# nhcha6/embodied-object-detection

Hardware: AMD Instinct MI355X
Metric: frames/sec (640x640, implicit_memory); frames/sec/GPU = value / n_gpus (higher is better)
Workload: dtype f32

## Files before the change

embodied_object_detection_amd/csrc/conv_common.h:

```cpp
#pragma once
#include "eod_common.h"
#include "../../include/eod_hip.h"

namespace eodconv {


struct ConvArgs {
  const float* x;
  const float* w;
  const float* bias;
  const float* res;
  const float* gate;
  float* y;
  float* partial;
  const int* m_count;
  int m_unit;
  int m_segs, seg_rows;
  const float* fuse_w;
  const int* out_units;
  float fuse_b;
  int N, H, W, Cin, OH, OW, Cout, KH, KW, stride, pad, Kpad;
  int M, nchunks, splitk, cps;
  int relu, res_mode, in_relu, out_mode;
  int tiles_m, tiles_n;
  float out_scale;
  int nlv;
  int lv_off[EOD_MAX_LEVELS + 1], lv_h[EOD_MAX_LEVELS], lv_w[EOD_MAX_LEVELS];
  unsigned x_bytes, w_bytes;
  const void* w3;
  unsigned w3_bytes;
  const void* wh;
  unsigned wh_bytes;
  double* gn_partial;
  int gn_groups;
  float* y2;
  int split_n;
  FastDiv div_ow, div_oh, div_cd, div_row;
};

__device__ __forceinline__ int conv_row_limit(const ConvArgs& p, int M) {
  if (p.m_count && p.m_segs <= 1) {
    const int lim = *p.m_count * p.m_unit;
    M = lim < M ? lim : M;
  }
  return M;
}

__device__ __forceinline__ bool conv_row_active(const ConvArgs& p, int m) {
  if (!p.m_count || p.m_segs <= 1) return true;
  const int s = m / p.seg_rows;
  return m - s * p.seg_rows < p.m_count[s] * p.m_unit;
}

__device__ __forceinline__ bool conv_tile_active(const ConvArgs& p, int m0, int bm) {
  if (!p.m_count || p.m_segs <= 1) return true;
  const int last = (m0 + bm - 1 < p.M ? m0 + bm - 1 : p.M - 1);
  const int s0 = m0 / p.seg_rows, s1 = last / p.seg_rows;
  if (m0 - s0 * p.seg_rows < p.m_count[s0] * p.m_unit) return true;
  for (int s = s0 + 1; s <= s1; ++s)
    if (p.m_count[s] > 0) return true;
  return false;
}

template <bool GATE = false>
__device__ __forceinline__ float epilogue_store(const ConvArgs& p, float v, int m, int n) {
  int co = n;
  size_t oidx;
  if (p.out_mode == 1) {
    const int Cd = p.Cout >> 2;
    const int quad = (int)fdiv((unsigned)n, p.div_cd);
    co = n - quad * Cd;
    const int dy = quad >> 1, dx = quad & 1;
    const int t = (int)fdiv((unsigned)m, p.div_ow);
    const int ox = m - t * p.OW;
    const int img = (int)fdiv((unsigned)t, p.div_oh);
    const int oy = t - img * p.OH;
    oidx = ((size_t)(img * 2 * p.OH + 2 * oy + dy) * (2 * p.OW) + (2 * ox + dx)) * Cd + co;
  } else {
    oidx = (size_t)m * p.Cout + n;
  }
  if (p.bias) v += p.bias[co];
  v *= p.out_scale;
  if (p.res_mode == 1) {
    v += p.res[(size_t)m * p.Cout + n];
  } else if (p.res_mode == 2) {
    const int t = (int)fdiv((unsigned)m, p.div_ow);
    const int ox = m - t * p.OW;
    const int img = (int)fdiv((unsigned)t, p.div_oh);
    const int oy = t - img * p.OH;
    const int rh = p.OH >> 1, rw = p.OW >> 1;
    v += p.res[((size_t)(img * rh + (oy >> 1)) * rw + (ox >> 1)) * p.Cout + n];
  }
  if (p.split_n > 0) {
    if (n >= p.split_n) {
      if (p.relu) v = fmaxf(v, 0.0f);
      p.y2[(size_t)m * (p.Cout - p.split_n) + (n - p.split_n)] = v;
    } else {
      p.y[(size_t)m * p.split_n + n] = v;
    }
    return v;
  }
  if (p.relu) v = fmaxf(v, 0.0f);
  if (GATE && p.gate && !(p.gate[oidx] > 0.0f)) v = 0.0f;
  p.y[oidx] = v;
  return v;
}

__device__ __forceinline__ unsigned long long tap_mask(int iy0, int ix0, int hh, int ww, int KH, int KW) {
  unsigned long long mask = 0;
  int tp = 0;
  for (int ky = 0; ky < KH; ++ky) {
    const bool rok = (unsigned)(iy0 + ky) < (unsigned)hh;
    for (int kx = 0; kx < KW; ++kx, ++tp) {
      const bool ok = rok && ((unsigned)(ix0 + kx) < (unsigned)ww);
      mask |= (unsigned long long)ok << tp;
    }
  }
  return mask;
}

template <int TM, int TN, bool GATE = false>
__device__ __forceinline__ void store_wave_tiles(const ConvArgs& p, const f32x16 (&acc)[TM][TN], int m_base, int n_base, int M, int z,
                                                 int lane) {
  const int half = lane >> 5;
#pragma unroll
  for (int i = 0; i < TM; ++i) {
#pragma unroll
    for (int j = 0; j < TN; ++j) {
      const int n = n_base + j * 32 + (lane & 31);
#pragma unroll
      for (int r = 0; r < 16; ++r) {
        const int row = (r & 3) + 8 * (r >> 2) + 4 * half;
        const int m = m_base + i * 32 + row;
        if (m < M && n < p.Cout && conv_row_active(p, m)) {
          const float v = acc[i][j][r];
          if (p.splitk > 1) {
            p.partial[((size_t)z * p.M + m) * p.Cout + n] = v;
          } else {
            epilogue_store<GATE>(p, v, m, n);
          }
        }
      }
    }
  }
}

void launch_conv_fp32(const ConvArgs& a, int tile, int bk, bool tap4, dim3 grid, hipStream_t s, int lds_reserve = 0, int prefetch2 = 0);
void launch_conv_bf16x3(const ConvArgs& a, int tile, dim3 grid, hipStream_t s);
void launch_conv_wavek(const ConvArgs& a, int nw, dim3 grid, hipStream_t s);
void launch_split_weights(const float* w, void* out, int Cout, int Kpad, hipStream_t s);
void launch_conv_f16(const ConvArgs& a, int tile, int bk, dim3 grid, hipStream_t s);
void launch_half_weights(const float* w, void* out, int Cout, int Kpad, hipStream_t s);

}
```

embodied_object_detection_amd/csrc/conv_fp32.hip:

```cpp
#include "conv_operands.h"

namespace eodconv {
namespace {

template <int BM, int BN, int BK, bool TAP4, bool MULTI, int PIPE = 0>
__global__ __launch_bounds__(256) void conv_igemm_kernel(ConvArgs p) {
  constexpr bool PF2 = PIPE == 1;
  constexpr bool DB = PIPE == 2;
  constexpr int LS = BK + 4;
  constexpr int TM = BM / 64, TN = BN / 64;
  constexpr int QPR = BK / 4;
  constexpr int RPP = 256 / QPR;
  constexpr int AR = BM / RPP, BR = BN / RPP;
  static_assert(!TAP4 || BK == 32, "the stem path stages one 7x7 tap per float4: BK must be 32");
  constexpr int BUF = (BM + BN) * LS;
  __shared__ __attribute__((aligned(16))) float lds[(DB ? 2 : 1) * BUF];
  float* As = lds;
  float* Bs = lds + BM * LS;

  const int tid = threadIdx.x;
  const int lane = tid & 63;
  const int wave = tid >> 6;
  const int wm = wave >> 1, wn = wave & 1;

  int M;
  const int t = conv_first_tile<BM>(p, M);
  if (t < 0) return;
  const int tile_m = t / p.tiles_n;
  const int tile_n = t - tile_m * p.tiles_n;
  const int m0 = tile_m * BM, n0 = tile_n * BN;
  if (!conv_tile_active(p, m0, BM)) return;
  const int z = blockIdx.y;
  int c_end;
  const int c_begin = conv_chunk_range(p, p.cps, z, c_end);

  const int lr = tid / QPR, lq = tid % QPR;
  int a_off[AR], a_iy[AR], a_ix[AR];
  unsigned a_voff[AR];
  unsigned long long a_mask[AR];
  unsigned a_pitch[MULTI ? AR : 1];
#pragma unroll
  for (int i = 0; i < AR; ++i) {
    const int m = m0 + lr + RPP * i;
    const bool rowok = m < M;
    const RowOrigin o = conv_row_origin<MULTI>(p, m, rowok);
    a_iy[i] = rowok ? o.iy0 : -(1 << 28);
    a_ix[i] = o.ix0;
    a_off[i] = o.off;
    if (!TAP4) conv_row_address<MULTI>(p, o, rowok, lq, a_voff[i], a_mask[i], a_pitch[MULTI ? i : 0]);
  }
  unsigned w_voff[BR];
#pragma unroll
  for (int j = 0; j < BR; ++j) w_voff[j] = conv_w_row_offset(p, n0 + lr + RPP * j, lq);
  const __amdgpu_buffer_rsrc_t rsrc_x = conv_buffer(p.x, p.x_bytes);
  const __amdgpu_buffer_rsrc_t rsrc_w = conv_buffer(p.w, p.w_bytes);

  f32x4 ar0[AR], br0[BR];
  f32x4 ar1[PF2 ? AR : 1], br1[PF2 ? BR : 1];
  ChunkWalker<BK, MULTI> walk(p, c_begin);
  auto load_chunk = [&](int chunk, auto& ar, auto& br) {
    const int k0 = chunk * BK;
    if (!TAP4) {
      const TapInfo ti = walk.next(p);
#pragma unroll
      for (int i = 0; i < AR; ++i) ar[i] = conv_load_a<MULTI>(rsrc_x, ti, a_voff[i], a_mask[i], a_pitch[MULTI ? i : 0]);
    } else {
      const int tap = chunk * 8 + lq;
      const int ky = tap / p.KW;
      const int kx = tap - ky * p.KW;
      const bool tv = tap < p.KH * p.KW;
#pragma unroll
      for (int i = 0; i < AR; ++i) {
        const int iy = a_iy[i] + ky, ix = a_ix[i] + kx;
        const bool ok = tv && ((unsigned)iy < (unsigned)p.H) && ((unsigned)ix < (unsigned)p.W);
        f32x4 v = {0.f, 0.f, 0.f, 0.f};
        if (ok) v = *reinterpret_cast<const f32x4*>(p.x + (size_t)(a_off[i] + iy * p.W + ix) * 4);
        ar[i] = v;
      }
    }
    if (p.in_relu) {
#pragma unroll
      for (int i = 0; i < AR; ++i) ar[i] = conv_relu4(ar[i]);
    }
#pragma unroll
    for (int j = 0; j < BR; ++j)
      br[j] = __builtin_bit_cast(f32x4, __builtin_amdgcn_raw_buffer_load_b128(rsrc_w, w_voff[j], k0 * 4, 0));
  };

  f32x16 acc[TM][TN];
#pragma unroll
  for (int i = 0; i < TM; ++i)
#pragma unroll
    for (int j = 0; j < TN; ++j)
#pragma unroll
      for (int r = 0; r < 16; ++r) acc[i][j][r] = 0.f;
  f32x16 acc_b;
#pragma unroll
// ... 8 lines not shown
#pragma unroll
    for (int kk = 0; kk < BK / 8; ++kk) {
      f32x4 af[TM], bf[TN];
#pragma unroll
      for (int i = 0; i < TM; ++i) af[i] = *reinterpret_cast<const f32x4*>(ab + i * 32 * LS + kk * 8);
#pragma unroll
      for (int j = 0; j < TN; ++j) bf[j] = *reinterpret_cast<const f32x4*>(bb + j * 32 * LS + kk * 8);
      __builtin_amdgcn_s_setprio(1);
#pragma unroll
      for (int tt = 0; tt < 4; ++tt)
#pragma unroll
        for (int i = 0; i < TM; ++i)
#pragma unroll
          for (int j = 0; j < TN; ++j)
            if (TM * TN == 1 && (tt & 1))
              acc_b = __builtin_amdgcn_mfma_f32_32x32x2f32(af[i][tt], bf[j][tt], acc_b, 0, 0, 0);
            else
              acc[i][j] = __builtin_amdgcn_mfma_f32_32x32x2f32(af[i][tt], bf[j][tt], acc[i][j], 0, 0, 0);
      __builtin_amdgcn_s_setprio(0);
    }
  };
  auto stage_and_multiply = [&](auto& ar, auto& br, int next_chunk) {
#pragma unroll
    for (int i = 0; i < AR; ++i) *reinterpret_cast<f32x4*>(As + (lr + RPP * i) * LS + 4 * lq) = ar[i];
#pragma unroll
    for (int j = 0; j < BR; ++j) *reinterpret_cast<f32x4*>(Bs + (lr + RPP * j) * LS + 4 * lq) = br[j];
    __syncthreads();
    if (next_chunk < c_end) load_chunk(next_chunk, ar, br);
    if constexpr (TM * TN == 1) {
      f32x4 af[2], bf[2];
      af[0] = *reinterpret_cast<const f32x4*>(a_base);
      bf[0] = *reinterpret_cast<const f32x4*>(b_base);
#pragma unroll
      for (int kk = 0; kk < BK / 8; ++kk) {
        const int cur = kk & 1, nxt = cur ^ 1;
        if (kk + 1 < BK / 8) {
          af[nxt] = *reinterpret_cast<const f32x4*>(a_base + (kk + 1) * 8);
          bf[nxt] = *reinterpret_cast<const f32x4*>(b_base + (kk + 1) * 8);
        }
        __builtin_amdgcn_s_setprio(1);
#pragma unroll
        for (int tt = 0; tt < 4; ++tt)
          if (tt & 1)
            acc_b = __builtin_amdgcn_mfma_f32_32x32x2f32(af[cur][tt], bf[cur][tt], acc_b, 0, 0, 0);
          else
            acc[0][0] = __builtin_amdgcn_mfma_f32_32x32x2f32(af[cur][tt], bf[cur][tt], acc[0][0], 0, 0, 0);
        __builtin_amdgcn_s_setprio(0);
      }
    } else {
      multiply(a_base, b_base);
    }
    __syncthreads();
  };
  load_chunk(c_begin, ar0, br0);
  if constexpr (DB) {
    auto store_tiles = [&](int buf) {
#pragma unroll
      for (int i = 0; i < AR; ++i) *reinterpret_cast<f32x4*>(As + buf * BUF + (lr + RPP * i) * LS + 4 * lq) = ar0[i];
#pragma unroll
      for (int j = 0; j < BR; ++j) *reinterpret_cast<f32x4*>(Bs + buf * BUF + (lr + RPP * j) * LS + 4 * lq) = br0[j];
    };
    store_tiles(0);
    __syncthreads();
    int cur = 0;
    for (int chunk = c_begin; chunk < c_end; ++chunk) {
      const bool more = chunk + 1 < c_end;
      if (more) load_chunk(chunk + 1, ar0, br0);
      multiply(a_base + cur * BUF, b_base + cur * BUF);
      if (more) store_tiles(cur ^ 1);
      __syncthreads();
      cur ^= 1;
    }
  } else if constexpr (PF2) {
    if (c_begin + 1 < c_end) load_chunk(c_begin + 1, ar1, br1);
    for (int chunk = c_begin; chunk < c_end; chunk += 2) {
      stage_and_multiply(ar0, br0, chunk + 2);
      if (chunk + 1 < c_end) stage_and_multiply(ar1, br1, chunk + 3);
    }
  } else {
    for (int chunk = c_begin; chunk < c_end; ++chunk) stage_and_multiply(ar0, br0, chunk + 1);
  }

  if (TM * TN == 1) {
#pragma unroll
    for (int r = 0; r < 16; ++r) acc[0][0][r] += acc_b[r];
  }
  if constexpr (BM == 64 && BN == 256) {
    if (p.out_mode == 2) {
      float sred[16];
#pragma unroll
      for (int r = 0; r < 16; ++r) sred[r] = 0.f;
#pragma unroll
      for (int j = 0; j < TN; ++j) {
        const int co = (wn * TN + j) * 32 + (lane & 31);
        const float bw = p.bias ? p.bias[co] : 0.f;
        const float pw = p.fuse_w[co];
#pragma unroll
        for (int r = 0; r < 16; ++r) {
          float v = (acc[0][j][r] + bw) * p.out_scale;
          if (p.relu) v = fmaxf(v, 0.f);
          sred[r] += v * pw;
        }
      }
#pragma unroll
      for (int off = 16; off > 0; off >>= 1)
#pragma unroll
        for (int r = 0; r < 16; ++r) sred[r] += __shfl_xor(sred[r], off, 64);
      float* red = lds;
      if ((lane & 31) == 0) {
        const int half = lane >> 5;
#pragma unroll
        for (int r = 0; r < 16; ++r) red[(wm * 2 + wn) * 32 + (r & 3) + 8 * (r >> 2) + 4 * half] = sred[r];
      }
      __syncthreads();
      if (tid < BM) {
        const int wr = tid >> 5, rr = tid & 31;
        const float v = red[(wr * 2 + 0) * 32 + rr] + red[(wr * 2 + 1) * 32 + rr] + p.fuse_b;
        const int m = m0 + tid;
        if (m < M) {
          const int tq = (int)fdiv((unsigned)m, p.div_ow);
          const int ox = m - tq * p.OW;
          const int img = (int)fdiv((unsigned)tq, p.div_oh);
          const int oy = tq - img * p.OH;
          const int unit = p.out_units ? p.out_units[img] : img;
          const int dy = tile_n >> 1, dx = tile_n & 1;
          p.y[((size_t)unit * 2 * p.OH + 2 * oy + dy) * (2 * p.OW) + 2 * ox + dx] = eod_sigmoid_precise(v);
        }
      }
      return;
    }
  }
  store_wave_tiles<TM, TN, BM == 64 && BN == 64>(p, acc, m0 + wm * TM * 32, n0 + wn * TN * 32, M, z, lane);
}


template <int NW, bool MULTI>
__global__ __launch_bounds__(NW * 64) void conv_wavek_kernel(ConvArgs p) {
  constexpr int BK = 32;
  constexpr int LS = BK + 4;
  constexpr int AR = 4;
  __shared__ __attribute__((aligned(16))) float lds[NW * 2 * 32 * LS];
  const int tid = threadIdx.x;
  const int lane = tid & 63;
  const int wave = tid >> 6;
  float* As = lds + wave * (2 * 32 * LS);
  float* Bs = As + 32 * LS;

  int M;
  const int t = conv_first_tile<32>(p, M);
  if (t < 0) return;
  const int tile_m = t / p.tiles_n;
  const int tile_n = t - tile_m * p.tiles_n;
  const int m0 = tile_m * 32, n0 = tile_n * 32;
  if (!conv_tile_active(p, m0, 32)) return;

  int c_end;
  const int c_begin = conv_chunk_range(p, (p.nchunks + NW - 1) / NW, wave, c_end);

  const int lr = lane >> 3, lq = lane & 7;
  unsigned a_voff[AR];
  unsigned long long a_mask[AR];
  unsigned a_pitch[MULTI ? AR : 1];
  unsigned w_voff[AR];
#pragma unroll
  for (int i = 0; i < AR; ++i) {
    conv_row_address<MULTI>(p, m0 + lr + 8 * i, M, lq, a_voff[i], a_mask[i], a_pitch[MULTI ? i : 0]);
    w_voff[i] = conv_w_row_offset(p, n0 + lr + 8 * i, lq);
  }
  const __amdgpu_buffer_rsrc_t rsrc_x = conv_buffer(p.x, p.x_bytes);
  const __amdgpu_buffer_rsrc_t rsrc_w = conv_buffer(p.w, p.w_bytes);

  f32x4 ar0[AR], br0[AR], ar1[AR], br1[AR];
  ChunkWalker<BK, MULTI> walk(p, c_begin);
  auto load_chunk = [&](int chunk, f32x4 (&ar)[AR], f32x4 (&br)[AR]) {
    const int k0 = chunk * BK;
    const TapInfo ti = walk.next(p);
#pragma unroll
    for (int i = 0; i < AR; ++i) ar[i] = conv_load_a<MULTI>(rsrc_x, ti, a_voff[i], a_mask[i], a_pitch[MULTI ? i : 0]);
    if (p.in_relu) {
#pragma unroll
      for (int i = 0; i < AR; ++i) ar[i] = conv_relu4(ar[i]);
    }
#pragma unroll
    for (int j = 0; j < AR; ++j)
      br[j] = __builtin_bit_cast(f32x4, __builtin_amdgcn_raw_buffer_load_b128(rsrc_w, w_voff[j], k0 * 4, 0));
// ... 26 lines not shown
      acc = __builtin_amdgcn_mfma_f32_32x32x2f32(af[0], bf[0], acc, 0, 0, 0);
      acc_b = __builtin_amdgcn_mfma_f32_32x32x2f32(af[1], bf[1], acc_b, 0, 0, 0);
      acc = __builtin_amdgcn_mfma_f32_32x32x2f32(af[2], bf[2], acc, 0, 0, 0);
      acc_b = __builtin_amdgcn_mfma_f32_32x32x2f32(af[3], bf[3], acc_b, 0, 0, 0);
    }
    __builtin_amdgcn_fence(__ATOMIC_RELEASE, "wavefront");
    __builtin_amdgcn_wave_barrier();
    __builtin_amdgcn_fence(__ATOMIC_ACQUIRE, "wavefront");
  };
  if (c_begin < c_end) load_chunk(c_begin, ar0, br0);
  if (c_begin + 1 < c_end) load_chunk(c_begin + 1, ar1, br1);
  for (int chunk = c_begin; chunk < c_end; chunk += 2) {
    stage_and_multiply(ar0, br0, chunk + 2);
    if (chunk + 1 < c_end) stage_and_multiply(ar1, br1, chunk + 3);
  }
#pragma unroll
  for (int r = 0; r < 16; ++r) acc[r] += acc_b[r];

  __syncthreads();
  float* red = lds;
  if (wave > 0) {
#pragma unroll
    for (int r = 0; r < 16; ++r) red[((wave - 1) * 16 + r) * 64 + lane] = acc[r];
  }
  __syncthreads();
  if (wave != 0) return;
#pragma unroll
  for (int w = 1; w < NW; ++w)
#pragma unroll
    for (int r = 0; r < 16; ++r) acc[r] += red[((w - 1) * 16 + r) * 64 + lane];
  f32x16 out[1][1];
  out[0][0] = acc;
  store_wave_tiles<1, 1, true>(p, out, m0, n0, M, 0, lane);
}

}

template <int BM, int BN>
static void launch_fp32_tile(const ConvArgs& a, bool tap4, int bk, dim3 grid, hipStream_t s, int dyn) {
  if (tap4)
    hipLaunchKernelGGL((conv_igemm_kernel<BM, BN, 32, true, false>), grid, dim3(256), dyn, s, a);
  else if (a.nlv > 0 && bk == 64)
    hipLaunchKernelGGL((conv_igemm_kernel<BM, BN, 64, false, true>), grid, dim3(256), dyn, s, a);
  else if (a.nlv > 0)
    hipLaunchKernelGGL((conv_igemm_kernel<BM, BN, 32, false, true>), grid, dim3(256), dyn, s, a);
  else if (bk == 64)
    hipLaunchKernelGGL((conv_igemm_kernel<BM, BN, 64, false, false>), grid, dim3(256), dyn, s, a);
  else
    hipLaunchKernelGGL((conv_igemm_kernel<BM, BN, 32, false, false>), grid, dim3(256), dyn, s, a);
}

void launch_conv_fp32(const ConvArgs& a, int tile, int bk, bool tap4, dim3 grid, hipStream_t s, int lds_reserve, int prefetch2) {
  const int dyn = lds_reserve > 0 ? lds_reserve : 0;
  if (prefetch2 == 1 && !tap4 && a.nlv == 0 && bk == 32 && tile == 3) {
    hipLaunchKernelGGL((conv_igemm_kernel<64, 64, 32, false, false, 1>), grid, dim3(256), dyn, s, a);
    return;
  }
  if (prefetch2 == 2 && !tap4 && bk == 32 && tile == 3) {
    if (a.nlv > 0) hipLaunchKernelGGL((conv_igemm_kernel<64, 64, 32, false, true, 2>), grid, dim3(256), dyn, s, a);
    else hipLaunchKernelGGL((conv_igemm_kernel<64, 64, 32, false, false, 2>), grid, dim3(256), dyn, s, a);
    return;
  }
  switch (tile) {
    case 5: hipLaunchKernelGGL((conv_igemm_kernel<64, 256, 32, false, false>), grid, dim3(256), dyn, s, a); break;
    case 1: launch_fp32_tile<128, 128>(a, tap4, bk, grid, s, dyn); break;
    case 2: launch_fp32_tile<128, 64>(a, tap4, bk, grid, s, dyn); break;
    default: launch_fp32_tile<64, 64>(a, tap4, bk, grid, s, dyn); break;
  }
}

void launch_conv_wavek(const ConvArgs& a, int nw, dim3 grid, hipStream_t s) {
  if (a.nlv > 0) {
    if (nw == 8) hipLaunchKernelGGL((conv_wavek_kernel<8, true>), grid, dim3(512), 0, s, a);
    else hipLaunchKernelGGL((conv_wavek_kernel<4, true>), grid, dim3(256), 0, s, a);
  } else {
    if (nw == 8) hipLaunchKernelGGL((conv_wavek_kernel<8, false>), grid, dim3(512), 0, s, a);
    else hipLaunchKernelGGL((conv_wavek_kernel<4, false>), grid, dim3(256), 0, s, a);
  }
}

}
```

embodied_object_detection_amd/csrc/conv_igemm.hip:

```cpp
#include "conv_common.h"
#include "../../include/eod_hip.h"
#include <atomic>
#include <cstdlib>
#include <cstring>

namespace {

using namespace eodconv;

template <int VEC>
__global__ __launch_bounds__(256) void conv_splitk_reduce_kernel(ConvArgs p) {
  EOD_CHAIN_PRIO();
  const int M = conv_row_limit(p, p.M);
  const unsigned per_row = (unsigned)p.Cout / VEC;
  const unsigned total = (unsigned)M * per_row;
  const size_t slab = (size_t)p.M * p.Cout;
  for (unsigned idx = blockIdx.x * blockDim.x + threadIdx.x; idx < total; idx += gridDim.x * blockDim.x) {
    const unsigned m = fdiv(idx, p.div_row);
    if (!conv_row_active(p, (int)m)) continue;
    const unsigned n = (idx - m * per_row) * VEC;
    const float* src = p.partial + (size_t)m * p.Cout + n;
    if (VEC == 4) {
      f32x4 v = {0.f, 0.f, 0.f, 0.f};
      for (int zb = 0; zb < p.splitk; zb += 4) {
// ... 128 lines not shown
  if (d->gate) {
    const bool f16_gated = d->math == EOD_MATH_F16 + 1 && half_ok && d->levels <= 0 && (d->force_tile == 0 || f16_forced);
    pick = 2;
    pl.glds = f16_gated ? 3 : 0;
  }
  if (pl.glds == 3) pl.bk = (fbk == 8 && d->Cin % 64 == 0) ? 64 : 32;
  else pl.bk = (pl.glds == 0 && d->out_mode != 2 && fbk == 2 && bk64_ok) ? 64 : 32;
  const int nchunks = d->Kpad / pl.bk;
  pl.nchunks = nchunks;
  pl.tile = pick + 1;
  pl.bm = cfg[pick][0];
  pl.bn = cfg[pick][1];
  pl.tiles_m = (M + pl.bm - 1) / pl.bm;
  pl.tiles_n = (d->Cout + pl.bn - 1) / pl.bn;
  const long tiles = (long)((Mp + pl.bm - 1) / pl.bm) * pl.tiles_n;
  int splitk = 1;
  if (d->out_mode == 2) {
    splitk = 1;
  } else if (d->force_splitk > 0) {
    splitk = d->force_splitk;
  } else if (pl.glds == 0 && !d->tap4 && nchunks >= 8 &&
             ((d->force_tile == 6 || d->force_tile == 7) ||
              (tiles < 256 && nchunks <= 192 && pl.bk == 32 && d->force_tile == 0 &&
               ((Mp <= 512 && nchunks / (nchunks >= 64 ? 8 : 4) >= 8) || nchunks >= 128)))) {
    pl.wavek = d->force_tile == 6 ? 4 : (d->force_tile == 7 ? 8 : (nchunks >= 64 ? 8 : 4));
    pl.bk = 32;
    pl.nchunks = d->Kpad / 32;
    pl.bm = pl.bn = 32;
    pl.tiles_m = (M + 31) / 32;
    pl.tiles_n = (d->Cout + 31) / 32;
  } else if (tiles < 256 && nchunks >= 8) {
    const int target = (nchunks >= 128 && Mp <= 512) ? 1792 : 512;
    int want = (int)((target + tiles - 1) / tiles);
    int maxs = nchunks / 4;
    splitk = want < maxs ? want : maxs;
    if (splitk < 1) splitk = 1;
  } else if (tiles >= 256 && tiles <= 1024 && d->m_count == nullptr && nchunks >= 18) {
    double best = 1e30;
    for (int sct = 1; sct <= 4; ++sct) {
      if (nchunks / sct < 9) break;
      const double est = (double)((tiles * sct + 255) / 256) / sct + (sct > 1 ? 0.12 : 0.0);
      if (est < best - 1e-9) {
        best = est;
        splitk = sct;
      }
    }
  }
  if (splitk > nchunks) splitk = nchunks;
  pl.cps = (nchunks + splitk - 1) / splitk;
  pl.splitk = (nchunks + pl.cps - 1) / pl.cps;
  return pl;
}

int total_rows(const EodConvDesc* d) { return d->levels > 0 ? d->level_off[d->levels] : d->N * d->OH * d->OW; }

int check_desc(const EodConvDesc* d) {
  if (!d || !d->x || !d->w || !d->y) return EOD_ERR_NULL;
  if (d->N <= 0 || d->Cin <= 0 || d->Cout <= 0) return EOD_ERR_BAD_DIMS;
  if (d->levels <= 0 && (d->H <= 0 || d->W <= 0 || d->OH <= 0 || d->OW <= 0)) return EOD_ERR_BAD_DIMS;
  if (d->KH <= 0 || d->KW <= 0 || d->stride <= 0 || d->pad < 0) return EOD_ERR_BAD_DIMS;
  if (d->Kpad % 32 != 0 || d->Kpad < d->KH * d->KW * d->Cin) return EOD_ERR_BAD_DIMS;
  if (d->tap4) {
    if (d->Cin != 4) return EOD_ERR_BAD_DIMS;
  } else {
    if (d->Cin % 32 != 0 || d->Kpad != d->KH * d->KW * d->Cin) return EOD_ERR_BAD_DIMS;
  }
  if (d->levels > 0) {
    if (d->levels > EOD_MAX_LEVELS || d->N != 1 || d->stride != 1 || d->KH != d->KW || d->pad != d->KH / 2 || d->tap4 || d->out_mode != 0 ||
        d->res_mode == 2 || d->level_off[0] != 0)
      return EOD_ERR_BAD_DIMS;
    for (int l = 0; l < d->levels; ++l)
      if (d->level_h[l] <= 0 || d->level_w[l] <= 0 || d->level_off[l + 1] - d->level_off[l] != d->level_h[l] * d->level_w[l])
        return EOD_ERR_BAD_DIMS;
  } else {
    if (d->OH != (d->H + 2 * d->pad - d->KH) / d->stride + 1) return EOD_ERR_BAD_DIMS;
    if (d->OW != (d->W + 2 * d->pad - d->KW) / d->stride + 1) return EOD_ERR_BAD_DIMS;
  }
  if (d->levels <= 0 && (long)d->N * d->H * d->W * d->Cin >= (1L << 29)) return EOD_ERR_BAD_DIMS;
  if ((long)d->Cout * d->Kpad >= (1L << 29)) return EOD_ERR_BAD_DIMS;
  if (d->KH * d->KW > 64) return EOD_ERR_BAD_DIMS;
  if ((long)total_rows(d) * (d->Cout > d->Cin ? d->Cout : d->Cin) >= (1L << 31)) return EOD_ERR_BAD_DIMS;
  if (d->out_mode == 1 && (d->Cout % 4 != 0)) return EOD_ERR_BAD_DIMS;
  if (d->out_mode == 2) {
    if (d->Cout != 1024 || d->KH != 1 || d->KW != 1 || d->stride != 1 || d->tap4 || d->levels > 0 || d->res_mode != 0 || d->in_relu ||
        d->force_splitk > 1)
      return EOD_ERR_BAD_DIMS;
    if (!d->fuse_w) return EOD_ERR_NULL;
  }
  if (d->out_mode < 0 || d->out_mode > 2) return EOD_ERR_BAD_DIMS;
  if (d->res_mode != 0 && !d->res) return EOD_ERR_NULL;
  if (d->res_mode == 2 && ((d->OH & 1) || (d->OW & 1))) return EOD_ERR_BAD_DIMS;
  if (d->m_count && d->m_unit <= 0) return EOD_ERR_BAD_DIMS;
  if (d->m_segments > 1) {
    if (!d->m_count || d->levels > 0 || d->out_mode == 2 || d->m_segments > EOD_MAX_BATCH || d->N % d->m_segments != 0)
      return EOD_ERR_BAD_DIMS;
    if (((long)(d->N / d->m_segments) * d->OH * d->OW) % d->m_unit != 0) return EOD_ERR_BAD_DIMS;
  }
  if (d->gate && (d->out_mode != 0 || d->split_n != 0 || d->gn_partial)) return EOD_ERR_BAD_DIMS;
  if (d->gate && d->force_tile != 0 && d->force_tile % 10 != 3 && d->force_tile != 6 && d->force_tile != 7) return EOD_ERR_BAD_DIMS;
  if (d->gate && d->force_tile / 10 == 5) return EOD_ERR_BAD_DIMS;
  if (d->gate && (d->force_tile / 10 == 8 || d->force_tile / 10 == 9) &&
      (d->math != EOD_MATH_F16 + 1 || d->force_tile % 10 != 3 || d->levels > 0 || d->tap4 || d->in_relu))
    return EOD_ERR_BAD_DIMS;
  if (d->math < 0 || d->math > EOD_MATH_F16 + 1) return EOD_ERR_BAD_DIMS;
  if ((d->force_tile / 10 == 8 || d->force_tile / 10 == 9) && d->force_tile % 10 != 3 && d->force_tile % 10 != 4) return EOD_ERR_BAD_DIMS;
  if (d->lds_reserve < 0 || d->lds_reserve > 48 * 1024) return EOD_ERR_BAD_DIMS;
// ... 68 lines not shown

extern "C" size_t eod_conv2d_workspace_bytes(const EodConvDesc* d) {
  if (check_desc(d) != EOD_OK) return 0;
  const int M = total_rows(d);
  const Plan pl = make_plan(d, M);
  if (pl.splitk <= 1) return 0;
  return (size_t)pl.splitk * M * d->Cout * sizeof(float);
}

extern "C" int eod_conv2d(const EodConvDesc* d, eod_stream_t stream) {
  const int st = check_desc(d);
  if (st != EOD_OK) return st;
  hipStream_t s = static_cast<hipStream_t>(stream);
  ConvArgs a{};
  a.x = d->x; a.w = d->w; a.bias = d->bias; a.res = d->res; a.y = d->y;
  a.partial = d->workspace;
  a.m_count = d->m_count; a.m_unit = d->m_unit;
  a.m_segs = d->m_segments > 1 ? d->m_segments : 1;
  a.seg_rows = a.m_segs > 1 ? (d->N / d->m_segments) * d->OH * d->OW : 0;
  a.fuse_w = d->fuse_w; a.out_units = d->out_units; a.fuse_b = d->fuse_b;
  a.N = d->N; a.H = d->H; a.W = d->W; a.Cin = d->Cin; a.OH = d->OH; a.OW = d->OW; a.Cout = d->Cout;
  a.KH = d->KH; a.KW = d->KW; a.stride = d->stride; a.pad = d->pad; a.Kpad = d->Kpad;
  a.M = total_rows(d);
  a.div_ow = eod_make_fastdiv((unsigned)(d->OW > 0 ? d->OW : 1));
  a.div_oh = eod_make_fastdiv((unsigned)(d->OH > 0 ? d->OH : 1));
  a.div_row = eod_make_fastdiv((unsigned)(d->Cout % 4 == 0 ? d->Cout / 4 : d->Cout));
  a.div_cd = eod_make_fastdiv((unsigned)((d->Cout >> 2) > 0 ? (d->Cout >> 2) : 1));
  {
    const size_t xe = d->levels > 0 ? (size_t)d->level_off[d->levels] * d->Cin : (size_t)d->N * d->H * d->W * d->Cin;
    a.x_bytes = (unsigned)(xe * sizeof(float));
    a.w_bytes = (unsigned)((size_t)d->Cout * d->Kpad * sizeof(float));
    a.w3 = d->w_split;
    a.w3_bytes = (unsigned)((size_t)d->Cout * d->Kpad * 6);
    a.wh = d->w_half;
    a.wh_bytes = (unsigned)((size_t)d->Cout * d->Kpad * 2);
  }
  a.nlv = d->levels > 0 ? d->levels : 0;
  for (int l = 0; l < a.nlv; ++l) {
    a.lv_off[l] = d->level_off[l];
    a.lv_h[l] = d->level_h[l];
    a.lv_w[l] = d->level_w[l];
  }
  if (a.nlv) a.lv_off[a.nlv] = d->level_off[a.nlv];
  a.relu = d->relu; a.res_mode = d->res_mode; a.in_relu = d->in_relu; a.out_mode = d->out_mode;
  a.gate = d->gate;
  a.out_scale = d->out_scale;
  a.gn_partial = d->gn_partial;
  a.gn_groups = d->gn_groups;
  a.y2 = d->y2;
  a.split_n = d->split_n;
  const Plan pl = make_plan(d, a.M);
  if (d->gn_partial && pl.splitk <= 1) return EOD_ERR_BAD_DIMS;
  a.nchunks = pl.nchunks;
  a.splitk = pl.splitk; a.cps = pl.cps; a.tiles_m = pl.tiles_m; a.tiles_n = pl.tiles_n;
  if (pl.splitk > 1) {
    const size_t need = (size_t)pl.splitk * a.M * a.Cout * sizeof(float);
    if (!d->workspace || d->workspace_bytes < need) return EOD_ERR_CAPACITY;
  }
  dim3 grid(pl.tiles_m * pl.tiles_n, pl.splitk);
  if (pl.wavek) launch_conv_wavek(a, pl.wavek, grid, s);
  else if (pl.glds == 3) launch_conv_f16(a, pl.tile, pl.bk, grid, s);
  else if (pl.glds == 2) launch_conv_bf16x3(a, pl.tile, grid, s);
  else launch_conv_fp32(a, pl.tile, pl.bk, d->tap4 != 0, grid, s, d->lds_reserve, d->prefetch2);
  if (pl.splitk > 1) {
    const size_t total = (size_t)a.M * a.Cout;
    const bool vec = a.Cout % 4 == 0;
    int blocks = (int)((total / (vec ? 4 : 1) + 255) / 256);
    if (blocks > 2048) blocks = 2048;
    if (blocks < 1) blocks = 1;
    if (a.gn_partial) {
      int chunks = 0;
      for (int l = 0; l < a.nlv; ++l) chunks += (a.lv_off[l + 1] - a.lv_off[l] + EOD_GN_ROWS - 1) / EOD_GN_ROWS;
      hipLaunchKernelGGL(conv_splitk_reduce_gn_kernel, dim3(chunks), dim3(256), 0, s, a);
    } else if (vec) hipLaunchKernelGGL(conv_splitk_reduce_kernel<4>, dim3(blocks), dim3(256), 0, s, a);
    else hipLaunchKernelGGL(conv_splitk_reduce_kernel<1>, dim3(blocks), dim3(256), 0, s, a);
  }
  return eod_launch_status();
}
```

embodied_object_detection_amd/csrc/conv_operands.h:

```cpp
#pragma once
#include "conv_common.h"

namespace eodconv {

template <int BM>
__device__ __forceinline__ int conv_first_tile(const ConvArgs& p, int& M) {
  M = conv_row_limit(p, p.M);
  const int ntiles = ((M + BM - 1) / BM) * p.tiles_n;
  if ((int)blockIdx.x >= ntiles) return -1;
  return xcd_remap(blockIdx.x, ntiles);
}

__device__ __forceinline__ int conv_chunk_range(const ConvArgs& p, int per, int idx, int& c_end) {
  const int c_begin = idx * per;
  c_end = c_begin + per;
  if (c_end > p.nchunks) c_end = p.nchunks;
  return c_begin;
}

struct RowOrigin {
  int iy0, ix0, off, hh, ww;
};
template <bool MULTI>
__device__ __forceinline__ RowOrigin conv_row_origin(const ConvArgs& p, int m, bool rowok) {
  RowOrigin o = {0, 0, 0, 1, 1};
  if (rowok) {
    if (MULTI) {
      int l = 0;
      while (l + 1 < p.nlv && m >= p.lv_off[l + 1]) ++l;
      const int local = m - p.lv_off[l];
      o.ww = p.lv_w[l];
      o.hh = p.lv_h[l];
      const int oy = local / o.ww;
      o.iy0 = oy - p.pad;
      o.ix0 = (local - oy * o.ww) - p.pad;
      o.off = p.lv_off[l];
    } else {
      const int t = (int)fdiv((unsigned)m, p.div_ow);
      const int ox = m - t * p.OW;
      const int img = (int)fdiv((unsigned)t, p.div_oh);
      const int oy = t - img * p.OH;
      o.iy0 = oy * p.stride - p.pad;
      o.ix0 = ox * p.stride - p.pad;
      o.off = img * p.H * p.W;
      o.hh = p.H;
      o.ww = p.W;
    }
  }
  return o;
}

template <bool MULTI>
__device__ __forceinline__ void conv_row_address(const ConvArgs& p, const RowOrigin& o, bool rowok, int lq, unsigned& voff,
                                                 unsigned long long& mask, unsigned& pitch) {
  mask = rowok ? tap_mask(o.iy0, o.ix0, o.hh, o.ww, p.KH, p.KW) : 0ull;
  voff = (unsigned)(((o.off + o.iy0 * o.ww + o.ix0) * p.Cin + 4 * lq) * 4);
  if (MULTI) pitch = (unsigned)(o.ww * p.Cin * 4);
}
template <bool MULTI>
__device__ __forceinline__ void conv_row_address(const ConvArgs& p, int m, int M, int lq, unsigned& voff, unsigned long long& mask,
                                                 unsigned& pitch) {
  const bool rowok = m < M;
  conv_row_address<MULTI>(p, conv_row_origin<MULTI>(p, m, rowok), rowok, lq, voff, mask, pitch);
}

__device__ __forceinline__ unsigned conv_w_row_offset(const ConvArgs& p, int n, int lq) {
  return n < p.Cout ? (unsigned)((n * p.Kpad + 4 * lq) * 4) : 0xFFFFFFFFu;
}

__device__ __forceinline__ __amdgpu_buffer_rsrc_t conv_buffer(const void* ptr, unsigned bytes) {
  return __builtin_amdgcn_make_buffer_rsrc(const_cast<void*>(ptr), 0, bytes, 0x00020000);
}

struct TapInfo {
  int tap, ky;
  unsigned tap_off, k0b;
};

template <int BK, bool MULTI>
struct ChunkWalker {
  int tap, c0, ky, kx, k0;
  __device__ __forceinline__ ChunkWalker(const ConvArgs& p, int c_begin) {
    k0 = c_begin * BK;
    tap = k0 / p.Cin;
    c0 = k0 - tap * p.Cin;
    ky = tap / p.KW;
    kx = tap - ky * p.KW;
  }
  __device__ __forceinline__ TapInfo next(const ConvArgs& p) {
    TapInfo ti;
    ti.tap = tap < 63 ? tap : 63;
    ti.ky = ky;
    ti.tap_off = MULTI ? (unsigned)((kx * p.Cin + c0) * 4) : (unsigned)(((ky * p.W + kx) * p.Cin + c0) * 4);
    ti.k0b = (unsigned)(k0 * 4);
    k0 += BK;
    c0 += BK;
    if (c0 >= p.Cin) {
      c0 = 0;
      ++tap;
      if (++kx == p.KW) {
        kx = 0;
        ++ky;
      }
    }
    return ti;
  }
};

template <bool MULTI>
__device__ __forceinline__ f32x4 conv_load_a(__amdgpu_buffer_rsrc_t rsrc_x, const TapInfo& ti, unsigned voff, unsigned long long mask,
                                             unsigned pitch) {
  const bool ok = (mask >> ti.tap) & 1ull;
  unsigned vo = voff + ti.tap_off;
  if (MULTI) vo += (unsigned)ti.ky * pitch;
  vo = ok ? vo : 0xFFFFFFFFu;
  return __builtin_bit_cast(f32x4, __builtin_amdgcn_raw_buffer_load_b128(rsrc_x, vo, 0, 0));
}

__device__ __forceinline__ f32x4 conv_relu4(f32x4 v) {
  v.x = fmaxf(v.x, 0.f);
  v.y = fmaxf(v.y, 0.f);
  v.z = fmaxf(v.z, 0.f);
  v.w = fmaxf(v.w, 0.f);
  return v;
}

}
```

embodied_object_detection_amd/build.py:

```python
from __future__ import annotations

import os
import subprocess
import sys

HERE = os.path.dirname(os.path.abspath(__file__))
CSRC = os.path.join(HERE, "csrc")
LIB = os.path.join(HERE, "libeod_hip.so")
SOURCES = ["conv_igemm.hip", "conv_fp32.hip", "conv_bf16x3.hip", "conv_f16.hip", "elementwise.hip", "roi_align.hip", "select.hip", "heads.hip", "memory.hip", "memory_read.hip", "memory_backward.hip", "conv_wgrad.hip", "train_losses.hip"]
ARCH = "gfx950"


def _stale() -> bool:
    if not os.path.exists(LIB):
        return True
    t = os.path.getmtime(LIB)
    deps = [os.path.join(CSRC, f) for f in os.listdir(CSRC)] + [os.path.join(HERE, "..", "include", "eod_hip.h")]
    return any(os.path.getmtime(d) > t for d in deps if os.path.exists(d))


def _usage_file(src: str) -> str:
    return os.path.join(HERE, "build", src.replace(".hip", ".usage.txt"))


def resource_usage() -> dict:
    import re
    out = {}
    for src in SOURCES:
        f = _usage_file(src)
        if not os.path.exists(f):
            continue
        cur = None
        for line in open(f):
            m = re.search(r"Function Name: (\S+)", line)
            if m:
                cur = out.setdefault(m.group(1), {})
                continue
            for key, pat in (("vgprs", r"\bVGPRs: (\d+)"), ("scratch", r"ScratchSize \[bytes/lane\]: (\d+)"),
                             ("occupancy", r"Occupancy \[waves/SIMD\]: (\d+)"), ("lds", r"LDS Size \[bytes/block\]: (\d+)")):
                m = re.search(pat, line)
                if m and cur is not None:
                    cur[key] = int(m.group(1))
    return out


def scratch_offenders(usage: dict = None) -> list:
    usage = resource_usage() if usage is None else usage
    return sorted(k for k, v in usage.items() if v.get("scratch", 0) > 0)


def build(force: bool = False, verbose: bool = True) -> str:
    if not force and not _stale():
        return LIB
    hipcc = os.environ.get("HIPCC", "/opt/rocm/bin/hipcc")
    objs = []
    procs = []
    os.makedirs(os.path.join(HERE, "build"), exist_ok=True)
    for src in SOURCES:
        obj = os.path.join(HERE, "build", src.replace(".hip", ".o"))
        cmd = [hipcc, f"--offload-arch={ARCH}", "-O3", "-fPIC", "-std=c++17", "-Wall", "-Wno-unused-function",
               "-ffp-contract=on", "-Rpass-analysis=kernel-resource-usage", "-c", os.path.join(CSRC, src), "-o", obj]
        if verbose:
            print(" ".join(cmd), flush=True)
        procs.append((src, subprocess.Popen(cmd, stderr=open(_usage_file(src), "w"))))
        objs.append(obj)
    failed = [s for s, p in procs if p.wait() != 0]
    for src in SOURCES:
        skip = 0
        for line in open(_usage_file(src)):
            if "kernel-resource-usage" in line:
                skip = 2 if "Function Name" in line else 0
                continue
            if skip and (line.lstrip()[:1].isdigit() or line.strip().startswith("|")):
                skip -= 1
                continue
            skip = 0
            if line.strip():
                sys.stderr.write(line)
    if failed:
        raise RuntimeError(f"hipcc failed for {failed}")
    bad = scratch_offenders()
    if bad:
        raise RuntimeError("kernels that use scratch memory (register spills / an argument struct copied to private memory): " + ", ".join(bad))
    cmd = [hipcc, f"--offload-arch={ARCH}", "-shared", "-fPIC", "-o", LIB] + objs
    if verbose:
        print(" ".join(cmd), flush=True)
    subprocess.check_call(cmd)
    return LIB


if __name__ == "__main__":
# ... 3 lines not shown
```

Baseline: 299.9.

## Reorder 3x3 conv rows border-first and skip padded taps per tile

For stride-1 pad-1 3x3 convs on plain images, output rows are permuted so that all border pixels come first (top/bottom rows, left/right columns) and interior pixels follow. Each 64-row tile ORs the tap-validity masks of its rows and skips K-chunks whose tap is out of bounds for every row, so border tiles avoid loading and multiplying zero-padding contributions. Stores go through an LDS row map back to the original indices. The cost is a prologue that computes the map and a sync, scattered stores, and loss of spatial locality in input loads. Only border tiles, a small fraction of the work, gain anything.

```diff
diff --git a/embodied_object_detection_amd/csrc/conv_common.h b/embodied_object_detection_amd/csrc/conv_common.h
--- a/embodied_object_detection_amd/csrc/conv_common.h
+++ b/embodied_object_detection_amd/csrc/conv_common.h
@@ -36,6 +36,8 @@
   float* y2;
   int split_n;
   FastDiv div_ow, div_oh, div_cd, div_row;
+  int border;
+  FastDiv div_bh, div_bw, div_bi;
 };
 
 __device__ __forceinline__ int conv_row_limit(const ConvArgs& p, int M) {
@@ -119,9 +121,9 @@
   return mask;
 }
 
-template <int TM, int TN, bool GATE = false>
+template <int TM, int TN, bool GATE = false, bool MAPPED = false>
 __device__ __forceinline__ void store_wave_tiles(const ConvArgs& p, const f32x16 (&acc)[TM][TN], int m_base, int n_base, int M, int z,
-                                                 int lane) {
+                                                 int lane, const int* row_map = nullptr) {
   const int half = lane >> 5;
 #pragma unroll
   for (int i = 0; i < TM; ++i) {
@@ -131,8 +133,9 @@
 #pragma unroll
       for (int r = 0; r < 16; ++r) {
         const int row = (r & 3) + 8 * (r >> 2) + 4 * half;
-        const int m = m_base + i * 32 + row;
+        int m = m_base + i * 32 + row;
         if (m < M && n < p.Cout && conv_row_active(p, m)) {
+          if (MAPPED) m = row_map[i * 32 + row];
           const float v = acc[i][j][r];
           if (p.splitk > 1) {
             p.partial[((size_t)z * p.M + m) * p.Cout + n] = v;
diff --git a/embodied_object_detection_amd/csrc/conv_fp32.hip b/embodied_object_detection_amd/csrc/conv_fp32.hip
--- a/embodied_object_detection_amd/csrc/conv_fp32.hip
+++ b/embodied_object_detection_amd/csrc/conv_fp32.hip
@@ -7,6 +7,8 @@
 __global__ __launch_bounds__(256) void conv_igemm_kernel(ConvArgs p) {
   constexpr bool PF2 = PIPE == 1;
   constexpr bool DB = PIPE == 2;
+  constexpr bool BORDER = PIPE == 3;
+  static_assert(!BORDER || (BM == 64 && BN == 64 && !TAP4 && !MULTI), "border-major order: the plain-image 64x64 tile only");
   constexpr int LS = BK + 4;
   constexpr int TM = BM / 64, TN = BN / 64;
   constexpr int QPR = BK / 4;
@@ -14,7 +16,7 @@
   constexpr int AR = BM / RPP, BR = BN / RPP;
   static_assert(!TAP4 || BK == 32, "the stem path stages one 7x7 tap per float4: BK must be 32");
   constexpr int BUF = (BM + BN) * LS;
-  __shared__ __attribute__((aligned(16))) float lds[(DB ? 2 : 1) * BUF];
+  __shared__ __attribute__((aligned(16))) float lds[(DB ? 2 : 1) * BUF + (BORDER ? BM + 4 : 0)];
   float* As = lds;
   float* Bs = lds + BM * LS;
 
@@ -35,14 +37,35 @@
   const int c_begin = conv_chunk_range(p, p.cps, z, c_end);
 
   const int lr = tid / QPR, lq = tid % QPR;
+  int* row_map = reinterpret_cast<int*>(lds + BUF);
+  unsigned tile_taps = 0;
+  if constexpr (BORDER) {
+    if (tid < BM) {
+      const int tr = m0 + tid;
+      int m = 0;
+      unsigned taps = 0;
+      if (tr < M) {
+        m = conv_border_row(p, tr, conv_border_count(p));
+        const RowOrigin o = conv_row_origin<false>(p, m, true);
+        taps = (unsigned)tap_mask(o.iy0, o.ix0, o.hh, o.ww, p.KH, p.KW);
+      }
+#pragma unroll
+      for (int off = 32; off > 0; off >>= 1) taps |= (unsigned)__shfl_xor((int)taps, off, 64);
+      row_map[tid] = m;
+      if (tid == 0) row_map[BM] = (int)taps;
+    }
+    __syncthreads();
+    tile_taps = (unsigned)__builtin_amdgcn_readfirstlane(row_map[BM]);
+  }
   int a_off[AR], a_iy[AR], a_ix[AR];
   unsigned a_voff[AR];
   unsigned long long a_mask[AR];
   unsigned a_pitch[MULTI ? AR : 1];
 #pragma unroll
   for (int i = 0; i < AR; ++i) {
-    const int m = m0 + lr + RPP * i;
-    const bool rowok = m < M;
+    const int tr = m0 + lr + RPP * i;
+    const bool rowok = tr < M;
+    const int m = BORDER ? row_map[lr + RPP * i] : tr;
     const RowOrigin o = conv_row_origin<MULTI>(p, m, rowok);
     a_iy[i] = rowok ? o.iy0 : -(1 << 28);
     a_ix[i] = o.ix0;
@@ -157,8 +180,20 @@
     }
     __syncthreads();
   };
-  load_chunk(c_begin, ar0, br0);
-  if constexpr (DB) {
+  if constexpr (BORDER) {
+    auto needed = [&](int c) {
+      while (c < c_end && !((tile_taps >> walk.tap) & 1u)) c += walk.seek_next_tap(p);
+      return c;
+    };
+    int chunk = needed(c_begin);
+    if (chunk < c_end) load_chunk(chunk, ar0, br0);
+    while (chunk < c_end) {
+      const int nc = needed(chunk + 1);
+      stage_and_multiply(ar0, br0, nc);
+      chunk = nc;
+    }
+  } else if constexpr (DB) {
+    load_chunk(c_begin, ar0, br0);
     auto store_tiles = [&](int buf) {
 #pragma unroll
       for (int i = 0; i < AR; ++i) *reinterpret_cast<f32x4*>(As + buf * BUF + (lr + RPP * i) * LS + 4 * lq) = ar0[i];
@@ -177,12 +212,14 @@
       cur ^= 1;
     }
   } else if constexpr (PF2) {
+    load_chunk(c_begin, ar0, br0);
     if (c_begin + 1 < c_end) load_chunk(c_begin + 1, ar1, br1);
     for (int chunk = c_begin; chunk < c_end; chunk += 2) {
       stage_and_multiply(ar0, br0, chunk + 2);
       if (chunk + 1 < c_end) stage_and_multiply(ar1, br1, chunk + 3);
     }
   } else {
+    load_chunk(c_begin, ar0, br0);
     for (int chunk = c_begin; chunk < c_end; ++chunk) stage_and_multiply(ar0, br0, chunk + 1);
   }
 
@@ -235,7 +272,10 @@
       return;
     }
   }
-  store_wave_tiles<TM, TN, BM == 64 && BN == 64>(p, acc, m0 + wm * TM * 32, n0 + wn * TN * 32, M, z, lane);
+  if constexpr (BORDER)
+    store_wave_tiles<TM, TN, true, true>(p, acc, m0 + wm * TM * 32, n0 + wn * TN * 32, M, z, lane, row_map + wm * TM * 32);
+  else
+    store_wave_tiles<TM, TN, BM == 64 && BN == 64>(p, acc, m0 + wm * TM * 32, n0 + wn * TN * 32, M, z, lane);
 }
 
 
@@ -368,6 +408,10 @@
 
 void launch_conv_fp32(const ConvArgs& a, int tile, int bk, bool tap4, dim3 grid, hipStream_t s, int lds_reserve, int prefetch2) {
   const int dyn = lds_reserve > 0 ? lds_reserve : 0;
+  if (a.border) {
+    hipLaunchKernelGGL((conv_igemm_kernel<64, 64, 32, false, false, 3>), grid, dim3(256), dyn, s, a);
+    return;
+  }
   if (prefetch2 == 1 && !tap4 && a.nlv == 0 && bk == 32 && tile == 3) {
     hipLaunchKernelGGL((conv_igemm_kernel<64, 64, 32, false, false, 1>), grid, dim3(256), dyn, s, a);
     return;
diff --git a/embodied_object_detection_amd/csrc/conv_igemm.hip b/embodied_object_detection_amd/csrc/conv_igemm.hip
--- a/embodied_object_detection_amd/csrc/conv_igemm.hip
+++ b/embodied_object_detection_amd/csrc/conv_igemm.hip
@@ -204,6 +204,12 @@
   return pl;
 }
 
+bool border_order(const EodConvDesc* d, const Plan& pl) {
+  return pl.glds == 0 && pl.wavek == 0 && pl.tile == 3 && pl.bk == 32 && d->prefetch2 == 0 && d->KH == 3 && d->KW == 3 &&
+         d->stride == 1 && d->pad == 1 && d->levels <= 0 && !d->tap4 && d->out_mode == 0 && d->split_n == 0 && d->m_count &&
+         d->m_segments <= 1 && d->m_unit == d->OH * d->OW && d->OH >= 3 && d->OW >= 3;
+}
+
 int total_rows(const EodConvDesc* d) { return d->levels > 0 ? d->level_off[d->levels] : d->N * d->OH * d->OW; }
 
 int check_desc(const EodConvDesc* d) {
@@ -378,6 +384,12 @@
   const Plan pl = make_plan(d, a.M);
   if (d->gn_partial && pl.splitk <= 1) return EOD_ERR_BAD_DIMS;
   a.nchunks = pl.nchunks;
+  if (border_order(d, pl)) {
+    a.border = 1;
+    a.div_bh = eod_make_fastdiv((unsigned)(d->OH - 2));
+    a.div_bw = eod_make_fastdiv((unsigned)(d->OW - 2));
+    a.div_bi = eod_make_fastdiv((unsigned)((d->OH - 2) * (d->OW - 2)));
+  }
   a.splitk = pl.splitk; a.cps = pl.cps; a.tiles_m = pl.tiles_m; a.tiles_n = pl.tiles_n;
   if (pl.splitk > 1) {
     const size_t need = (size_t)pl.splitk * a.M * a.Cout * sizeof(float);
diff --git a/embodied_object_detection_amd/csrc/conv_operands.h b/embodied_object_detection_amd/csrc/conv_operands.h
--- a/embodied_object_detection_amd/csrc/conv_operands.h
+++ b/embodied_object_detection_amd/csrc/conv_operands.h
@@ -48,6 +48,38 @@
     }
   }
   return o;
+}
+
+__device__ __forceinline__ int conv_border_count(const ConvArgs& p) {
+  const int n = *p.m_count;
+  return n < p.N ? n : p.N;
+}
+__device__ __forceinline__ int conv_border_row(const ConvArgs& p, int t, int count) {
+  const int bh = p.OH - 2, bw = p.OW - 2;
+  const int n_row = count * p.OW, n_col = count * bh;
+  int img, oy, ox;
+  if (t < 2 * n_row) {
+    const bool top = t < n_row;
+    const int u = top ? t : t - n_row;
+    img = (int)fdiv((unsigned)u, p.div_ow);
+    oy = top ? 0 : p.OH - 1;
+    ox = u - img * p.OW;
+  } else if (t < 2 * (n_row + n_col)) {
+    const int v = t - 2 * n_row;
+    const bool left = v < n_col;
+    const int u = left ? v : v - n_col;
+    img = (int)fdiv((unsigned)u, p.div_bh);
+    oy = 1 + u - img * bh;
+    ox = left ? 0 : p.OW - 1;
+  } else {
+    const int u = t - 2 * (n_row + n_col);
+    img = (int)fdiv((unsigned)u, p.div_bi);
+    const int r = u - img * bh * bw;
+    const int q = (int)fdiv((unsigned)r, p.div_bw);
+    oy = 1 + q;
+    ox = 1 + r - q * bw;
+  }
+  return (img * p.OH + oy) * p.OW + ox;
 }
 
 template <bool MULTI>
@@ -105,6 +137,17 @@
     }
     return ti;
   }
+  __device__ __forceinline__ int seek_next_tap(const ConvArgs& p) {
+    const int ahead = (p.Cin - c0) / BK;
+    k0 += p.Cin - c0;
+    c0 = 0;
+    ++tap;
+    if (++kx == p.KW) {
+      kx = 0;
+      ++ky;
+    }
+    return ahead;
+  }
 };
 
 template <bool MULTI>
```

New measurement: 298.1. About the same (-0.6%).

## Add dedicated 512-thread mask-tail conv kernel with split-wave fused reduction

Applied to the files above, without the earlier changes.

Replaces the generic 64x256 igemm instantiation used for tile 5 (the mask-head tail conv fused with the 1x1 projection and sigmoid) with a dedicated 8-wave kernel. Each wave holds only two 32x32 accumulators, loads are register-prefetched one chunk ahead, MFMA issue is wrapped in setprio, and the kernel requests 6 waves per EU. The fused epilogue is split so paired waves hand partial sums through LDS before the shuffle reduction. The aim is fewer registers and more latency hiding, paid for with an extra LDS handoff, an extra barrier, and a dedicated code path for tile 5. The build script also records AGPR counts.

```diff
diff --git a/embodied_object_detection_amd/build.py b/embodied_object_detection_amd/build.py
--- a/embodied_object_detection_amd/build.py
+++ b/embodied_object_detection_amd/build.py
@@ -36,7 +36,7 @@
             if m:
                 cur = out.setdefault(m.group(1), {})
                 continue
-            for key, pat in (("vgprs", r"\bVGPRs: (\d+)"), ("scratch", r"ScratchSize \[bytes/lane\]: (\d+)"),
+            for key, pat in (("vgprs", r"\bVGPRs: (\d+)"), ("agprs", r"\bAGPRs: (\d+)"), ("scratch", r"ScratchSize \[bytes/lane\]: (\d+)"),
                              ("occupancy", r"Occupancy \[waves/SIMD\]: (\d+)"), ("lds", r"LDS Size \[bytes/block\]: (\d+)")):
                 m = re.search(pat, line)
                 if m and cur is not None:
diff --git a/embodied_object_detection_amd/csrc/conv_fp32.hip b/embodied_object_detection_amd/csrc/conv_fp32.hip
--- a/embodied_object_detection_amd/csrc/conv_fp32.hip
+++ b/embodied_object_detection_amd/csrc/conv_fp32.hip
@@ -190,52 +190,145 @@
 #pragma unroll
     for (int r = 0; r < 16; ++r) acc[0][0][r] += acc_b[r];
   }
-  if constexpr (BM == 64 && BN == 256) {
-    if (p.out_mode == 2) {
-      float sred[16];
-#pragma unroll
-      for (int r = 0; r < 16; ++r) sred[r] = 0.f;
-#pragma unroll
-      for (int j = 0; j < TN; ++j) {
-        const int co = (wn * TN + j) * 32 + (lane & 31);
-        const float bw = p.bias ? p.bias[co] : 0.f;
-        const float pw = p.fuse_w[co];
-#pragma unroll
-        for (int r = 0; r < 16; ++r) {
-          float v = (acc[0][j][r] + bw) * p.out_scale;
-          if (p.relu) v = fmaxf(v, 0.f);
-          sred[r] += v * pw;
-        }
+  store_wave_tiles<TM, TN, BM == 64 && BN == 64>(p, acc, m0 + wm * TM * 32, n0 + wn * TN * 32, M, z, lane);
+}
+
+
+__global__ __launch_bounds__(512) __attribute__((amdgpu_waves_per_eu(6))) void conv_mask_tail_kernel(ConvArgs p) {
+  constexpr int BM = 64, BN = 256, BK = 32;
+  constexpr int LS = BK + 4;
+  constexpr int QPR = BK / 4;
+  constexpr int RPP = 512 / QPR;
+  constexpr int BR = BN / RPP;
+  constexpr int TN = 2;
+  static_assert(RPP == BM, "one A row per thread");
+  __shared__ __attribute__((aligned(16))) float lds[(BM + BN) * LS];
+  float* As = lds;
+  float* Bs = lds + BM * LS;
+
+  const int tid = threadIdx.x;
+  const int lane = tid & 63;
+  const int wave = tid >> 6;
+  const int wm = wave >> 2, w4 = wave & 3;
+
+  int M;
+  const int t = conv_first_tile<BM>(p, M);
+  if (t < 0) return;
+  const int tile_m = t / p.tiles_n;
+  const int tile_n = t - tile_m * p.tiles_n;
+  const int m0 = tile_m * BM, n0 = tile_n * BN;
+  if (!conv_tile_active(p, m0, BM)) return;
+
+  const int lr = tid / QPR, lq = tid % QPR;
+  unsigned a_voff, a_pitch;
+  unsigned long long a_mask;
+  conv_row_address<false>(p, m0 + lr, M, lq, a_voff, a_mask, a_pitch);
+  unsigned w_voff[BR];
+#pragma unroll
+  for (int j = 0; j < BR; ++j) w_voff[j] = conv_w_row_offset(p, n0 + lr + RPP * j, lq);
+  const __amdgpu_buffer_rsrc_t rsrc_x = conv_buffer(p.x, p.x_bytes);
+  const __amdgpu_buffer_rsrc_t rsrc_w = conv_buffer(p.w, p.w_bytes);
+
+  f32x4 ar, br[BR];
+  ChunkWalker<BK, false> walk(p, 0);
+  auto load_chunk = [&](int chunk) {
+    const TapInfo ti = walk.next(p);
+    ar = conv_load_a<false>(rsrc_x, ti, a_voff, a_mask, a_pitch);
+#pragma unroll
+    for (int j = 0; j < BR; ++j)
+      br[j] = __builtin_bit_cast(f32x4, __builtin_amdgcn_raw_buffer_load_b128(rsrc_w, w_voff[j], chunk * BK * 4, 0));
+  };
+
+  f32x16 acc[TN];
+#pragma unroll
+  for (int j = 0; j < TN; ++j)
+#pragma unroll
+    for (int r = 0; r < 16; ++r) acc[j][r] = 0.f;
+
+  const int frag_row = lane & 31;
+  const int frag_k = 4 * (lane >> 5);
+  const float* a_base = As + (wm * 32 + frag_row) * LS + frag_k;
+  const float* b_base = Bs + (w4 * TN * 32 + frag_row) * LS + frag_k;
+
+  load_chunk(0);
+  for (int chunk = 0; chunk < p.nchunks; ++chunk) {
+    *reinterpret_cast<f32x4*>(As + lr * LS + 4 * lq) = ar;
+#pragma unroll
+    for (int j = 0; j < BR; ++j) *reinterpret_cast<f32x4*>(Bs + (lr + RPP * j) * LS + 4 * lq) = br[j];
+    __syncthreads();
+    if (chunk + 1 < p.nchunks) load_chunk(chunk + 1);
+#pragma unroll
+    for (int kk = 0; kk < BK / 8; ++kk) {
+      f32x4 bf[TN];
+      const f32x4 af = *reinterpret_cast<const f32x4*>(a_base + kk * 8);
+#pragma unroll
+      for (int j = 0; j < TN; ++j) bf[j] = *reinterpret_cast<const f32x4*>(b_base + j * 32 * LS + kk * 8);
+      __builtin_amdgcn_s_setprio(1);
+#pragma unroll
+      for (int tt = 0; tt < 4; ++tt)
+#pragma unroll
+        for (int j = 0; j < TN; ++j) acc[j] = __builtin_amdgcn_mfma_f32_32x32x2f32(af[tt], bf[j][tt], acc[j], 0, 0, 0);
+      __builtin_amdgcn_s_setprio(0);
+    }
+    __syncthreads();
+  }
+
+  float* hand = lds;
+  float* red = lds + 4 * 16 * 64;
+  const int wn = w4 >> 1;
+  float* my_hand = hand + (wm * 2 + wn) * 16 * 64 + lane;
+  float sred[16];
+  auto lane_chain = [&]() {
+#pragma unroll
+    for (int j = 0; j < TN; ++j) {
+      const int co = (w4 * TN + j) * 32 + (lane & 31);
+      const float bw = p.bias ? p.bias[co] : 0.f;
+      const float pw = p.fuse_w[co];
+#pragma unroll
+      for (int r = 0; r < 16; ++r) {
+        float v = (acc[j][r] + bw) * p.out_scale;
+        if (p.relu) v = fmaxf(v, 0.f);
+        sred[r] += v * pw;
       }
-#pragma unroll
-      for (int off = 16; off > 0; off >>= 1)
-#pragma unroll
-        for (int r = 0; r < 16; ++r) sred[r] += __shfl_xor(sred[r], off, 64);
-      float* red = lds;
-      if ((lane & 31) == 0) {
-        const int half = lane >> 5;
-#pragma unroll
-        for (int r = 0; r < 16; ++r) red[(wm * 2 + wn) * 32 + (r & 3) + 8 * (r >> 2) + 4 * half] = sred[r];
-      }
-      __syncthreads();
-      if (tid < BM) {
-        const int wr = tid >> 5, rr = tid & 31;
-        const float v = red[(wr * 2 + 0) * 32 + rr] + red[(wr * 2 + 1) * 32 + rr] + p.fuse_b;
-        const int m = m0 + tid;
-        if (m < M) {
-          const int tq = (int)fdiv((unsigned)m, p.div_ow);
-          const int ox = m - tq * p.OW;
-          const int img = (int)fdiv((unsigned)tq, p.div_oh);
-          const int oy = tq - img * p.OH;
-          const int unit = p.out_units ? p.out_units[img] : img;
-          const int dy = tile_n >> 1, dx = tile_n & 1;
-          p.y[((size_t)unit * 2 * p.OH + 2 * oy + dy) * (2 * p.OW) + 2 * ox + dx] = eod_sigmoid_precise(v);
-        }
-      }
-      return;
-    }
-  }
-  store_wave_tiles<TM, TN, BM == 64 && BN == 64>(p, acc, m0 + wm * TM * 32, n0 + wn * TN * 32, M, z, lane);
+    }
+  };
+  if (!(w4 & 1)) {
+#pragma unroll
+    for (int r = 0; r < 16; ++r) sred[r] = 0.f;
+    lane_chain();
+#pragma unroll
+    for (int r = 0; r < 16; ++r) my_hand[r * 64] = sred[r];
+  }
+  __syncthreads();
+  if (w4 & 1) {
+#pragma unroll
+    for (int r = 0; r < 16; ++r) sred[r] = my_hand[r * 64];
+    lane_chain();
+#pragma unroll
+    for (int off = 16; off > 0; off >>= 1)
+#pragma unroll
+      for (int r = 0; r < 16; ++r) sred[r] += __shfl_xor(sred[r], off, 64);
+    if ((lane & 31) == 0) {
+      const int half = lane >> 5;
+#pragma unroll
+      for (int r = 0; r < 16; ++r) red[(wm * 2 + wn) * 32 + (r & 3) + 8 * (r >> 2) + 4 * half] = sred[r];
+    }
+  }
+  __syncthreads();
+  if (tid < BM) {
+    const int wr = tid >> 5, rr = tid & 31;
+    const float v = red[(wr * 2 + 0) * 32 + rr] + red[(wr * 2 + 1) * 32 + rr] + p.fuse_b;
+    const int m = m0 + tid;
+    if (m < M) {
+      const int tq = (int)fdiv((unsigned)m, p.div_ow);
+      const int ox = m - tq * p.OW;
+      const int img = (int)fdiv((unsigned)tq, p.div_oh);
+      const int oy = tq - img * p.OH;
+      const int unit = p.out_units ? p.out_units[img] : img;
+      const int dy = tile_n >> 1, dx = tile_n & 1;
+      p.y[((size_t)unit * 2 * p.OH + 2 * oy + dy) * (2 * p.OW) + 2 * ox + dx] = eod_sigmoid_precise(v);
+    }
+  }
 }
 
 
@@ -378,7 +471,7 @@
     return;
   }
   switch (tile) {
-    case 5: hipLaunchKernelGGL((conv_igemm_kernel<64, 256, 32, false, false>), grid, dim3(256), dyn, s, a); break;
+    case 5: hipLaunchKernelGGL(conv_mask_tail_kernel, grid, dim3(512), dyn, s, a); break;
     case 1: launch_fp32_tile<128, 128>(a, tap4, bk, grid, s, dyn); break;
     case 2: launch_fp32_tile<128, 64>(a, tap4, bk, grid, s, dyn); break;
     default: launch_fp32_tile<64, 64>(a, tap4, bk, grid, s, dyn); break;
```

New measurement: 298.9 before, 299.0 after (median of 2 runs). Within noise of the previous version (+0.0%).
